# SonyCSLParis/vqcpc-bach

Measured on AMD Instinct MI355X. Metric: encoder-train windows/sec (Bach 4-voice, seq=256), higher is better.
Workload: dtype f32

## Files before the change

### vqcpc_bach_amd/csrc/embed_ln.hip

```cpp
#include <stdlib.h>

#include "common.h"
#include "gemm_common.h"

namespace vq {

__global__ __launch_bounds__(256) void embed_pos_fwd_kernel(const int64_t* __restrict__ tokens, int64_t n_rows, int tpb,
                                                            int nv, const float* __restrict__ table, int vmax, int dlin,
                                                            const float* __restrict__ chan, const float* __restrict__ ev,
                                                            int pos, float* __restrict__ out) {
    const int d = dlin + (ev ? 2 : 1) * pos;
    const int d4 = d >> 2;
    const int64_t total = n_rows * d4;
    int64_t e = (int64_t)blockIdx.x * blockDim.x + threadIdx.x;
    const int64_t step = (int64_t)gridDim.x * blockDim.x;
    for (; e < total; e += step) {
        const int64_t row = e / d4;
        const int col = (int)(e - row * d4) << 2;
        const int p = (int)(row % tpb);
        const int v = p % nv, evt = p / nv;
        float4 val;
        if (col < dlin) {
            const int64_t tok = tokens[row];
            val = *reinterpret_cast<const float4*>(table + ((int64_t)v * vmax + tok) * dlin + col);
// ... 206 lines not shown
                    const float4 rv = nt_load4(r + row * d + col);
                    xv.x += rv.x * msk[it].x;
                    xv.y += rv.y * msk[it].y;
                    xv.z += rv.z * msk[it].z;
                    xv.w += rv.w * msk[it].w;
                }
                const float4 dv = DYB16 ? nt_load4_bf16(reinterpret_cast<const unsigned short*>(dy) + row * d + col)
                                        : nt_load4(dy + row * d + col);
                xh[it] = make_float4((xv.x - mu) * rs, (xv.y - mu) * rs, (xv.z - mu) * rs, (xv.w - mu) * rs);
                gy[it] = make_float4(dv.x * gm[it].x, dv.y * gm[it].y, dv.z * gm[it].z, dv.w * gm[it].w);
                s1 += (gy[it].x + gy[it].y) + (gy[it].z + gy[it].w);
                s2 += (gy[it].x * xh[it].x + gy[it].y * xh[it].y) + (gy[it].z * xh[it].z + gy[it].w * xh[it].w);
                dg[it].x += dv.x * xh[it].x;
                dg[it].y += dv.y * xh[it].y;
                dg[it].z += dv.z * xh[it].z;
                dg[it].w += dv.w * xh[it].w;
                db[it].x += dv.x;
                db[it].y += dv.y;
                db[it].z += dv.z;
                db[it].w += dv.w;
            }
        }
        const float m1 = wave_sum(s1) * inv_d, m2 = wave_sum(s2) * inv_d;
#pragma unroll
        for (int it = 0; it < NIT; ++it) {
            const int col = lane * 4 + it * 256;
            if (it < nit && col < d) {
                float4 o;
                o.x = rs * (gy[it].x - m1 - xh[it].x * m2);
                o.y = rs * (gy[it].y - m1 - xh[it].y * m2);
                o.z = rs * (gy[it].z - m1 - xh[it].z * m2);
                o.w = rs * (gy[it].w - m1 - xh[it].w * m2);
                if (d_s) nt_store4(d_s + row * d + col, o);
                if (ds_b16) *reinterpret_cast<uint2*>(ds_b16 + row * d + col) = round4_bf16(o);
                if (MASKED && (d_r != nullptr || dr_b16 != nullptr)) {
                    o.x *= msk[it].x;
                    o.y *= msk[it].y;
                    o.z *= msk[it].z;
                    o.w *= msk[it].w;
                    if (d_r != nullptr) nt_store4(d_r + row * d + col, o);
                }
                if (dr_b16) *reinterpret_cast<uint2*>(dr_b16 + row * d + col) = round4_bf16(o);
            }
        }
    }
#pragma unroll
    for (int it = 0; it < NIT; ++it) {
        const int col = lane * 4 + it * 256;
        if (it < nit && col < d) {
            *reinterpret_cast<float4*>(&red[(wave * 2 + 0) * kRedW + col]) = dg[it];
            *reinterpret_cast<float4*>(&red[(wave * 2 + 1) * kRedW + col]) = db[it];
        }
    }
    __syncthreads();
    for (int i = threadIdx.x; i < 2 * d; i += 256) {
        const int which = i / d, col = i % d;
        float acc = 0.0f;
#pragma unroll
        for (int w = 0; w < 4; ++w) acc += red[(w * 2 + which) * kRedW + col];
        ws[(int64_t)blockIdx.x * 2 * d + i] = acc;
    }
}

__global__ __launch_bounds__(256) void embed_pos_scatter_kernel(const float* __restrict__ tmp, int nv, int64_t tab, int pos,
                                                                int nev, float* __restrict__ d_table,
                                                                float* __restrict__ d_chan, float* __restrict__ d_event) {
    const int64_t per = tab + pos + (int64_t)nev * pos;
    const int64_t i = (int64_t)blockIdx.x * 256 + threadIdx.x;
    const int64_t n1 = (int64_t)nv * (tab + pos);
    if (i < n1) {
        const int v = (int)(i / (tab + pos));
        const int64_t j = i - (int64_t)v * (tab + pos);
        const float x = tmp[(int64_t)v * per + j];
        if (j < tab) d_table[(int64_t)v * tab + j] = x;
        else d_chan[(int64_t)v * pos + (j - tab)] = x;
    } else if (i < n1 + (int64_t)nev * pos) {
        const int64_t e = i - n1;
        float acc = 0.0f;
        for (int v = 0; v < nv; ++v) acc += tmp[(int64_t)v * per + tab + pos + e];
        d_event[e] = acc;
    }
}

static int ln_blocks(int64_t M) { return (int)std::min<int64_t>(ceil_div(M, 4), 2048); }
static int ln_bwd_blocks(int64_t M, bool has_r, int d) {
    static const int cap_env = lab_env_int("VQCPC_LN_BWD_BLOCKS", 0);
    const int cap = cap_env > 0 ? cap_env : ((has_r || d > 512) ? 512 : 1024);
    return (int)std::min<int64_t>(ceil_div(M, 4), cap);
}
static int ln_bwd_blocks_max(int64_t M, int d) { return std::max(ln_bwd_blocks(M, true, d), ln_bwd_blocks(M, false, d)); }

__global__ __launch_bounds__(256) void block_table_gather_kernel(const float* __restrict__ table,
                                                                 const int64_t* __restrict__ tokens,
                                                                 float* __restrict__ out, int64_t M, int L, int C4) {
    const int64_t total = M * C4;
    for (int64_t e = (int64_t)blockIdx.x * blockDim.x + threadIdx.x; e < total; e += (int64_t)gridDim.x * blockDim.x) {
        const int64_t r = e / C4;
        const int c = (int)(e - r * C4);
        const int64_t id = tokens[r] * L + (r % L);
        reinterpret_cast<float4*>(out)[e] = reinterpret_cast<const float4*>(table)[id * C4 + c];
    }
}

constexpr int kSegU = 32;

template <bool G16>
__global__ __launch_bounds__(256) void block_table_segsum_kernel(const float* __restrict__ g,
                                                                 const int64_t* __restrict__ tokens,
                                                                 float* __restrict__ ws, int64_t n_blocks,
                                                                 int blocks_per_chunk, int L, int vmax, int C) {
    constexpr int W = G16 ? 2 : 1;
    extern __shared__ __attribute__((aligned(16))) float acc[];
    for (int i = threadIdx.x; i < vmax * 256 * W; i += 256) acc[i] = 0.0f;
    __syncthreads();
    const int ctiles = (C + 256 * W - 1) / (256 * W);
    const int ct = blockIdx.x % ctiles, p = (blockIdx.x / ctiles) % L, chunk = blockIdx.x / (ctiles * L);
    const int col = (ct * 256 + threadIdx.x) * W;
    const bool cok = col < C;
    const int64_t b0 = (int64_t)chunk * blocks_per_chunk;
    const int64_t b1 = min(b0 + blocks_per_chunk, n_blocks);
    const float* gp = g + (cok ? col : 0);
    const unsigned short* gp16 = reinterpret_cast<const unsigned short*>(g) + (cok ? col : 0);
    float* mine = acc + threadIdx.x * W;
    static_assert(kSegU <= 64, "one lane per row of a batch holds its token");
    for (int64_t b = b0; b < b1; b += kSegU) {
        float v[kSegU][W];
        const int tokv = (int)tokens[min(b + (int)(threadIdx.x & 63) % kSegU, b1 - 1) * L + p];
#pragma unroll
        for (int u = 0; u < kSegU; ++u) {
            const int64_t row = min(b + u, b1 - 1) * L + p;
            if constexpr (G16) {
                const uint32_t t = *reinterpret_cast<const uint32_t*>(gp16 + row * C);
                v[u][0] = b + u < b1 ? __uint_as_float(t << 16) : 0.0f;
                v[u][W - 1] = b + u < b1 ? __uint_as_float(t & 0xFFFF0000u) : 0.0f;
            } else {
                v[u][0] = b + u < b1 ? gp[row * C] : 0.0f;
            }
        }
#pragma unroll
        for (int u = 0; u < kSegU; ++u) {
            float* cell = mine + __builtin_amdgcn_readlane(tokv, u) * (256 * W);
#pragma unroll
            for (int w = 0; w < W; ++w) cell[w] += v[u][w];
        }
    }
    __syncthreads();
    if (cok) {
        float* dst = ws + (int64_t)chunk * vmax * L * C;
        for (int t = 0; t < vmax; ++t)
#pragma unroll
            for (int w = 0; w < W; ++w) dst[((int64_t)t * L + p) * C + col + w] = acc[(t * 256 + threadIdx.x) * W + w];
    }
}

__global__ __launch_bounds__(256) void embedding_bwd_kernel(const float* __restrict__ g, int64_t ldg,
                                                            const int64_t* __restrict__ sorted_idx,
                                                            const int64_t* __restrict__ perm, float* __restrict__ d_table,
                                                            int64_t M, int C) {
    constexpr int U = 8;
    const int64_t m = blockIdx.x;
    const int64_t v = sorted_idx[m];
    if (m > 0 && sorted_idx[m - 1] == v) return;
    int64_t lo = m, hi = M;
    while (lo + 1 < hi) {
        const int64_t mid = (lo + hi) >> 1;
        if (sorted_idx[mid] == v) lo = mid; else hi = mid;
    }
// ... 290 lines not shown
```

### vqcpc_bach_amd/csrc/relattn16.hip

```cpp
#include "gemm_common.h"

namespace vq {

typedef float floatx4 __attribute__((ext_vector_type(4)));

constexpr int kA16Waves = 4;
constexpr int kA16RS = 33;

__device__ __forceinline__ const float* erel16(const float* __restrict__ e1, const float* __restrict__ e2, int h, int HD,
                                               int x) {
    x = min(x, 30);
    return x < 16 ? e1 + ((int64_t)h * 16 + x) * HD : e2 + ((int64_t)h * 16 + (x - 15)) * HD;
}

__device__ __forceinline__ void wave_lds_fence() {
    __builtin_amdgcn_fence(__ATOMIC_RELEASE, "wavefront");
    __builtin_amdgcn_wave_barrier();
    __builtin_amdgcn_fence(__ATOMIC_ACQUIRE, "wavefront");
}

template <int N>
__device__ __forceinline__ void load_f4(float (&dst)[N], const float* __restrict__ p, float mul) {
#pragma unroll
    for (int v = 0; v < N / 4; ++v) {
// ... 37 lines not shown
    else store_ct<CT>(base + off, v);
}


__device__ __forceinline__ float bf16_lo(uint32_t w) { return __uint_as_float(w << 16); }
__device__ __forceinline__ float bf16_hi(uint32_t w) { return __uint_as_float(w & 0xFFFF0000u); }
template <int N, bool IN16>
__device__ __forceinline__ void load_vec(float (&dst)[N], const float* __restrict__ base, int64_t off, float mul) {
    if constexpr (!IN16) {
        load_f4<N>(dst, base + off, mul);
    } else {
        const unsigned short* p = reinterpret_cast<const unsigned short*>(base) + off;
        if constexpr (N == 4) {
            const uint2 t = *reinterpret_cast<const uint2*>(p);
            dst[0] = bf16_lo(t.x) * mul; dst[1] = bf16_hi(t.x) * mul; dst[2] = bf16_lo(t.y) * mul; dst[3] = bf16_hi(t.y) * mul;
        } else {
#pragma unroll
            for (int v = 0; v < N / 8; ++v) {
                const uint4 t = *reinterpret_cast<const uint4*>(p + 8 * v);
                dst[8 * v] = bf16_lo(t.x) * mul; dst[8 * v + 1] = bf16_hi(t.x) * mul;
                dst[8 * v + 2] = bf16_lo(t.y) * mul; dst[8 * v + 3] = bf16_hi(t.y) * mul;
                dst[8 * v + 4] = bf16_lo(t.z) * mul; dst[8 * v + 5] = bf16_hi(t.z) * mul;
                dst[8 * v + 6] = bf16_lo(t.w) * mul; dst[8 * v + 7] = bf16_hi(t.w) * mul;
            }
        }
    }
}
template <int CT, bool IN16>
__device__ __forceinline__ void load_cols(float (&dst)[CT], const float* __restrict__ base, int64_t off, float mul) {
    if constexpr (!IN16) {
        load_ct<CT>(dst, base + off, mul);
    } else {
        const unsigned short* p = reinterpret_cast<const unsigned short*>(base) + off;
        if constexpr (CT == 4) {
            const uint2 t = *reinterpret_cast<const uint2*>(p);
            dst[0] = bf16_lo(t.x) * mul; dst[1] = bf16_hi(t.x) * mul; dst[2 % CT] = bf16_lo(t.y) * mul; dst[3 % CT] = bf16_hi(t.y) * mul;
        } else if constexpr (CT == 2) {
            const uint32_t t = *reinterpret_cast<const uint32_t*>(p);
            dst[0] = bf16_lo(t) * mul; dst[1 % CT] = bf16_hi(t) * mul;
        } else {
            dst[0] = __uint_as_float((uint32_t)p[0] << 16) * mul;
        }
    }
}

__device__ __forceinline__ void split8x3(const float (&x)[8], bf16x8& h, bf16x8& m, bf16x8& l) {
    uint2 h0, m0, l0, h1, m1, l1;
    split3x4(make_float4(x[0], x[1], x[2], x[3]), h0, m0, l0);
    split3x4(make_float4(x[4], x[5], x[6], x[7]), h1, m1, l1);
    h = __builtin_bit_cast(bf16x8, make_uint4(h0.x, h0.y, h1.x, h1.y));
    m = __builtin_bit_cast(bf16x8, make_uint4(m0.x, m0.y, m1.x, m1.y));
    l = __builtin_bit_cast(bf16x8, make_uint4(l0.x, l0.y, l1.x, l1.y));
}
__device__ __forceinline__ floatx4 dot32_x6(const bf16x8& ah, const bf16x8& am, const bf16x8& al, const bf16x8& bh,
                                            const bf16x8& bm, const bf16x8& bl, floatx4 acc) {
    acc = __builtin_amdgcn_mfma_f32_16x16x32_bf16(al, bh, acc, 0, 0, 0);
    acc = __builtin_amdgcn_mfma_f32_16x16x32_bf16(ah, bl, acc, 0, 0, 0);
    acc = __builtin_amdgcn_mfma_f32_16x16x32_bf16(am, bm, acc, 0, 0, 0);
    acc = __builtin_amdgcn_mfma_f32_16x16x32_bf16(am, bh, acc, 0, 0, 0);
    acc = __builtin_amdgcn_mfma_f32_16x16x32_bf16(ah, bm, acc, 0, 0, 0);
    acc = __builtin_amdgcn_mfma_f32_16x16x32_bf16(ah, bh, acc, 0, 0, 0);
    return acc;
}

__device__ __forceinline__ float grp16_sum(float v) {
    v += __shfl_xor(v, 1, 16); v += __shfl_xor(v, 2, 16); v += __shfl_xor(v, 4, 16); v += __shfl_xor(v, 8, 16);
    return v;
}
__device__ __forceinline__ float grp16_max(float v) {
    v = fmaxf(v, __shfl_xor(v, 1, 16)); v = fmaxf(v, __shfl_xor(v, 2, 16));
    v = fmaxf(v, __shfl_xor(v, 4, 16)); v = fmaxf(v, __shfl_xor(v, 8, 16));
    return v;
}

template <int HD, bool B16 = false, bool IN16 = false, bool X6 = false>
__global__ __launch_bounds__(kA16Waves * 64) void relattn16_fwd_kernel(const float* __restrict__ qkv, int64_t ldq,
                                                                       const int64_t* __restrict__ tokens,
                                                                       const float* __restrict__ e1,
                                                                       const float* __restrict__ e2, float* __restrict__ ctx,
                                                                       int64_t ldo, float* __restrict__ probs,
                                                                       int64_t total, int H, float scale, uint32_t thr,
                                                                       float inv_keep, uint64_t seed) {
    constexpr int KH = HD / 4, CT = HD / 16;
    __shared__ float lds[kA16Waves][16 * kA16RS];
    const int lane = threadIdx.x & 63, wave = threadIdx.x >> 6, g = lane >> 4, c = lane & 15;
    float* buf = lds[wave];
    const int64_t prob = min((int64_t)blockIdx.x * kA16Waves + wave, total - 1);
    const bool live = (int64_t)blockIdx.x * kA16Waves + wave < total;
    const int64_t n = prob / H;
    const int h = (int)(prob % H);
    const int d = H * HD;
    const int64_t tokv = tokens ? tokens[n * 16 + c] : 0;
    const int64_t row_c = tokens ? tokv * 16 + c : n * 16 + c;
    const int64_t ro = row_c * ldq + h * HD + g * KH;

    float qa[KH], kb[KH];
    load_vec<KH, IN16>(qa, qkv, ro, scale);
    load_vec<KH, IN16>(kb, qkv, ro + d, 1.0f);
    floatx4 s = {0.f, 0.f, 0.f, 0.f};
    if constexpr (X6 && (HD == 32 || HD == 64)) {
        constexpr int NCH = KH / 8;
        constexpr bool Q1 = IN16 && HD == 64, K1 = IN16;
        bf16x8 qh[NCH], qm[NCH], ql[NCH];
#pragma unroll
        for (int ch = 0; ch < NCH; ++ch) {
            float q8[8], k8[8];
#pragma unroll
            for (int k = 0; k < 8; ++k) { q8[k] = qa[8 * ch + k]; k8[k] = kb[8 * ch + k]; }
            bf16x8 kh_, km, kl;
            split8x3(q8, qh[ch], qm[ch], ql[ch]);
            split8x3(k8, kh_, km, kl);
            if constexpr (Q1 && K1) {
                s = __builtin_amdgcn_mfma_f32_16x16x32_bf16(qh[ch], kh_, s, 0, 0, 0);
            } else if constexpr (K1) {
                s = __builtin_amdgcn_mfma_f32_16x16x32_bf16(ql[ch], kh_, s, 0, 0, 0);
                s = __builtin_amdgcn_mfma_f32_16x16x32_bf16(qm[ch], kh_, s, 0, 0, 0);
                s = __builtin_amdgcn_mfma_f32_16x16x32_bf16(qh[ch], kh_, s, 0, 0, 0);
            } else {
                s = dot32_x6(qh[ch], qm[ch], ql[ch], kh_, km, kl, s);
            }
        }
#pragma unroll
        for (int t = 0; t < 2; ++t) {
            float eb[KH];
            load_f4<KH>(eb, erel16(e1, e2, h, HD, 16 * t + c) + g * KH, 1.0f);
            floatx4 qe = {0.f, 0.f, 0.f, 0.f};
#pragma unroll
            for (int ch = 0; ch < NCH; ++ch) {
                float e8[8];
#pragma unroll
                for (int k = 0; k < 8; ++k) e8[k] = eb[8 * ch + k];
                bf16x8 eh, em, el;
                split8x3(e8, eh, em, el);
                if constexpr (Q1) {
                    qe = __builtin_amdgcn_mfma_f32_16x16x32_bf16(qh[ch], el, qe, 0, 0, 0);
                    qe = __builtin_amdgcn_mfma_f32_16x16x32_bf16(qh[ch], em, qe, 0, 0, 0);
                    qe = __builtin_amdgcn_mfma_f32_16x16x32_bf16(qh[ch], eh, qe, 0, 0, 0);
                } else {
                    qe = dot32_x6(qh[ch], qm[ch], ql[ch], eh, em, el, qe);
                }
            }
#pragma unroll
            for (int r = 0; r < 4; ++r) buf[(4 * g + r) * kA16RS + 16 * t + c] = qe[r];
        }
    } else {
#pragma unroll
    for (int k = 0; k < KH; ++k) s = __builtin_amdgcn_mfma_f32_16x16x4f32(qa[k], kb[k], s, 0, 0, 0);
#pragma unroll
    for (int t = 0; t < 2; ++t) {
        float eb[KH];
        load_f4<KH>(eb, erel16(e1, e2, h, HD, 16 * t + c) + g * KH, 1.0f);
        floatx4 qe = {0.f, 0.f, 0.f, 0.f};
#pragma unroll
        for (int k = 0; k < KH; ++k) qe = __builtin_amdgcn_mfma_f32_16x16x4f32(qa[k], eb[k], qe, 0, 0, 0);
#pragma unroll
        for (int r = 0; r < 4; ++r) buf[(4 * g + r) * kA16RS + 16 * t + c] = qe[r];
    }
    }
    wave_lds_fence();
    float p[4], pd[4];
#pragma unroll
    for (int r = 0; r < 4; ++r) {
        const int i = 4 * g + r;
        const float v = s[r] + buf[i * kA16RS + c - i + 15];
        const float m = grp16_max(v);
        const float e = __expf(v - m);
        p[r] = e / grp16_sum(e);
        const int64_t idx = (prob * 16 + i) * 16 + c;
        if (live) probs[idx] = p[r];
        pd[r] = p[r] * drop_scale(seed, (uint64_t)idx, thr, inv_keep);
    }
    wave_lds_fence();
#pragma unroll
    for (int r = 0; r < 4; ++r) buf[(4 * g + r) * kA16RS + c] = pd[r];
    wave_lds_fence();
    floatx4 o[CT];
#pragma unroll
    for (int ct = 0; ct < CT; ++ct) o[ct] = floatx4{0.f, 0.f, 0.f, 0.f};
#pragma unroll
    for (int sidx = 0; sidx < 4; ++sidx) {
        const int j = 4 * g + sidx;
        const float pa = buf[c * kA16RS + j];
        const int64_t tj = __shfl(tokv, j, 16);
        const int64_t row_j = tokens ? tj * 16 + j : n * 16 + j;
        float vb[CT];
        load_cols<CT, IN16>(vb, qkv, row_j * ldq + 2 * d + h * HD + CT * c, 1.0f);
#pragma unroll
        for (int ct = 0; ct < CT; ++ct) o[ct] = __builtin_amdgcn_mfma_f32_16x16x4f32(pa, vb[ct], o[ct], 0, 0, 0);
    }
    if (live) {
#pragma unroll
        for (int r = 0; r < 4; ++r) {
            float v[CT];
#pragma unroll
            for (int ct = 0; ct < CT; ++ct) v[ct] = o[ct][r];
            store_out<CT, B16>(ctx, (n * 16 + 4 * g + r) * ldo + h * HD + CT * c, v);
        }
    }
}

template <int HD, bool B16 = false, bool IN16 = false>
__global__ __launch_bounds__(kA16Waves * 64) void relattn16_bwd_kernel(
    const float* __restrict__ d_ctx, int64_t ldo, const float* __restrict__ qkv, int64_t ldq,
    const int64_t* __restrict__ tokens, const float* __restrict__ probs, const float* __restrict__ e1,
    const float* __restrict__ e2, float* __restrict__ d_qkv, int64_t ldg, float* __restrict__ ws, int64_t n_blocks, int H,
    int blocks_per_chunk, float scale, uint32_t thr, float inv_keep, uint64_t seed) {
    constexpr int KH = HD / 4, CT = HD / 16;
    __shared__ float lds[kA16Waves][16 * kA16RS];
    const int lane = threadIdx.x & 63, wave = threadIdx.x >> 6, g = lane >> 4, c = lane & 15;
    float* buf = lds[wave];
    const int h = blockIdx.y;
    const int d = H * HD;
    floatx4 de[2][CT];
#pragma unroll
    for (int t = 0; t < 2; ++t)
#pragma unroll
        for (int ct = 0; ct < CT; ++ct) de[t][ct] = floatx4{0.f, 0.f, 0.f, 0.f};
    const int64_t b0 = (int64_t)blockIdx.x * blocks_per_chunk;
    const int64_t b1 = min(b0 + blocks_per_chunk, n_blocks);
    const int iters = (int)((b1 - b0 + kA16Waves - 1) / kA16Waves);
    constexpr bool kPipe = HD <= 32;
    struct Blk {
        float doa[KH], vb[KH], p[4], dob[4][CT], qb[4][CT], kb[4][CT];
    };
    auto block_of = [&](int it) { return min(b0 + (int64_t)it * kA16Waves + wave, b1 - 1); };
    auto load_tok = [&](int64_t n) -> int64_t { return tokens ? tokens[n * 16 + c] : 0; };
    auto load_blk = [&](Blk& B, int64_t n, int64_t tokv) {
        const int64_t prob = n * H + h;
        const int64_t row_c = tokens ? tokv * 16 + c : n * 16 + c;
        load_vec<KH, IN16>(B.doa, d_ctx, (n * 16 + c) * ldo + h * HD + g * KH, 1.0f);
        load_vec<KH, IN16>(B.vb, qkv, row_c * ldq + h * HD + 2 * d + g * KH, 1.0f);
#pragma unroll
        for (int r = 0; r < 4; ++r) B.p[r] = probs[(prob * 16 + 4 * g + r) * 16 + c];
#pragma unroll
        for (int sidx = 0; sidx < 4; ++sidx) {
            const int j = 4 * g + sidx;
            const int64_t tj = __shfl(tokv, j, 16);
            const int64_t row = tokens ? tj * 16 + j : n * 16 + j;
            load_cols<CT, IN16>(B.dob[sidx], d_ctx, (n * 16 + j) * ldo + h * HD + CT * c, 1.0f);
            load_cols<CT, IN16>(B.qb[sidx], qkv, row * ldq + h * HD + CT * c, scale);
            load_cols<CT, IN16>(B.kb[sidx], qkv, row * ldq + d + h * HD + CT * c, 1.0f);
        }
    };
    Blk cur;
    int64_t tok_n1 = 0;
    if (kPipe) {
        load_blk(cur, block_of(0), load_tok(block_of(0)));
        tok_n1 = load_tok(block_of(1));
    }
    for (int it = 0; it < iters; ++it) {
        const int64_t want = b0 + (int64_t)it * kA16Waves + wave;
        const bool live = want < b1;
        const int64_t n = live ? want : b1 - 1;
        const int64_t prob = n * H + h;
        Blk nxt;
        if (kPipe) {
            load_blk(nxt, block_of(it + 1), tok_n1);
            tok_n1 = load_tok(block_of(it + 2));
        } else {
            load_blk(cur, n, load_tok(n));
        }
        floatx4 dp = {0.f, 0.f, 0.f, 0.f};
#pragma unroll
        for (int k = 0; k < KH; ++k) dp = __builtin_amdgcn_mfma_f32_16x16x4f32(cur.doa[k], cur.vb[k], dp, 0, 0, 0);
        float pd[4], ds[4];
#pragma unroll
        for (int r = 0; r < 4; ++r) {
            const int64_t idx = (prob * 16 + 4 * g + r) * 16 + c;
            const float p = cur.p[r];
            const float mk = drop_scale(seed, (uint64_t)idx, thr, inv_keep);
            const float dpm = dp[r] * mk;
            pd[r] = p * mk;
            ds[r] = p * (dpm - grp16_sum(dpm * p));
        }
        floatx4 dv[CT], dk[CT], dq[CT];
#pragma unroll
        for (int ct = 0; ct < CT; ++ct) dv[ct] = dk[ct] = dq[ct] = floatx4{0.f, 0.f, 0.f, 0.f};
#pragma unroll
        for (int sidx = 0; sidx < 4; ++sidx) {
#pragma unroll
            for (int ct = 0; ct < CT; ++ct) {
                dv[ct] = __builtin_amdgcn_mfma_f32_16x16x4f32(pd[sidx], cur.dob[sidx][ct], dv[ct], 0, 0, 0);
                dk[ct] = __builtin_amdgcn_mfma_f32_16x16x4f32(ds[sidx], cur.qb[sidx][ct], dk[ct], 0, 0, 0);
            }
        }
        wave_lds_fence();
#pragma unroll
        for (int r = 0; r < 4; ++r) buf[(4 * g + r) * kA16RS + c] = ds[r];
        wave_lds_fence();
#pragma unroll
        for (int sidx = 0; sidx < 4; ++sidx) {
            const float a = buf[c * kA16RS + 4 * g + sidx];
#pragma unroll
            for (int ct = 0; ct < CT; ++ct)
                dq[ct] = __builtin_amdgcn_mfma_f32_16x16x4f32(a, cur.kb[sidx][ct], dq[ct], 0, 0, 0);
        }
#pragma unroll
        for (int xt = 0; xt < 2; ++xt)
#pragma unroll
            for (int sidx = 0; sidx < 4; ++sidx) {
                const int x = 16 * xt + 4 * g + sidx;
                const int jj = x + c - 15;
                const float a = (x <= 30 && jj >= 0 && jj < 16) ? buf[c * kA16RS + jj] : 0.0f;
                float eb2[CT];
                load_ct<CT>(eb2, erel16(e1, e2, h, HD, x) + CT * c, 1.0f);
#pragma unroll
                for (int ct = 0; ct < CT; ++ct) dq[ct] = __builtin_amdgcn_mfma_f32_16x16x4f32(a, eb2[ct], dq[ct], 0, 0, 0);
            }
        if (live) {
#pragma unroll
            for (int xt = 0; xt < 2; ++xt)
#pragma unroll
                for (int sidx = 0; sidx < 4; ++sidx) {
                    const int i = 4 * g + sidx, x = 16 * xt + c;
                    const int jj = x + i - 15;
                    const float a = (x <= 30 && jj >= 0 && jj < 16) ? buf[i * kA16RS + jj] : 0.0f;
#pragma unroll
                    for (int ct = 0; ct < CT; ++ct)
                        de[xt][ct] = __builtin_amdgcn_mfma_f32_16x16x4f32(a, cur.qb[sidx][ct], de[xt][ct], 0, 0, 0);
                }
#pragma unroll
            for (int r = 0; r < 4; ++r) {
                float vq[CT], vk[CT], vv[CT];
#pragma unroll
                for (int ct = 0; ct < CT; ++ct) {
                    vq[ct] = dq[ct][r] * scale;
                    vk[ct] = dk[ct][r];
                    vv[ct] = dv[ct][r];
                }
                const int64_t go = (n * 16 + 4 * g + r) * ldg + h * HD + CT * c;
                store_out<CT, B16>(d_qkv, go, vq);
                store_out<CT, B16>(d_qkv, go + d, vk);
                store_out<CT, B16>(d_qkv, go + 2 * d, vv);
            }
        }
        if (kPipe) cur = nxt;
    }
    float* dst = ws + (((int64_t)blockIdx.x * kA16Waves + wave) * H + h) * 31 * HD;
#pragma unroll
    for (int xt = 0; xt < 2; ++xt)
#pragma unroll
        for (int ct = 0; ct < CT; ++ct)
#pragma unroll
            for (int r = 0; r < 4; ++r) {
                const int x = 16 * xt + 4 * g + r;
                if (x <= 30) dst[x * HD + CT * c + ct] = de[xt][ct][r];
            }
}

__device__ __forceinline__ uint32_t perm_lo(uint32_t hi_src, uint32_t lo_src) { return __builtin_amdgcn_perm(hi_src, lo_src, 0x05040100u); }
__device__ __forceinline__ uint32_t perm_hi(uint32_t hi_src, uint32_t lo_src) { return __builtin_amdgcn_perm(hi_src, lo_src, 0x07060302u); }
__device__ __forceinline__ void split2x4(const float (&v)[4], uint32_t& h01, uint32_t& h23, uint32_t& l01, uint32_t& l23) {
    h01 = bf16x2_rn(v[0], v[1]);
    h23 = bf16x2_rn(v[2], v[3]);
    l01 = bf16x2_rn(v[0] - bf16_lo(h01), v[1] - bf16_hi(h01));
    l23 = bf16x2_rn(v[2] - bf16_lo(h23), v[3] - bf16_hi(h23));
}
__device__ __forceinline__ bf16x8 frag8(uint32_t a, uint32_t b, uint32_t c, uint32_t d) {
    return __builtin_bit_cast(bf16x8, make_uint4(a, b, c, d));
}
__device__ __forceinline__ bf16x8 frag_from_packed(uint32_t d0, uint32_t d1, uint32_t d2, uint32_t d3) {
    return frag8(perm_hi(d1, d0), perm_hi(d3, d2), perm_lo(d1, d0), perm_lo(d3, d2));
}
template <int CT>
__device__ __forceinline__ void tr_rows4(const uint32_t (&R)[4][CT / 2], uint32_t (&T)[CT][2]) {
#pragma unroll
    for (int w = 0; w < CT / 2; ++w) {
        T[2 * w][0] = perm_lo(R[1][w], R[0][w]);
        T[2 * w][1] = perm_lo(R[3][w], R[2][w]);
        T[2 * w + 1][0] = perm_hi(R[1][w], R[0][w]);
        T[2 * w + 1][1] = perm_hi(R[3][w], R[2][w]);
    }
}
template <int CT>
__device__ __forceinline__ void load_row_b16(uint32_t (&dst)[CT / 2], const unsigned short* __restrict__ p) {
    if constexpr (CT == 4) {
        const uint2 t = *reinterpret_cast<const uint2*>(p);
        dst[0] = t.x; dst[1 % (CT / 2)] = t.y;
    } else {
        dst[0] = *reinterpret_cast<const uint32_t*>(p);
    }
}

template <int HD>
__global__ __launch_bounds__(kA16Waves * 64, 2) void relattn16_bwd_mm16_kernel(
    const unsigned short* __restrict__ d_ctx, int64_t ldo, const unsigned short* __restrict__ qkv, int64_t ldq,
    const float* __restrict__ probs, const float* __restrict__ e1, const float* __restrict__ e2,
    unsigned short* __restrict__ d_qkv, int64_t ldg, float* __restrict__ ws, int64_t n_blocks, int H, int blocks_per_chunk,
    float scale, uint32_t thr, float inv_keep, uint64_t seed) {
    static_assert(HD == 32 || HD == 64, "head_dim 32 / 64");
    constexpr int KH = HD / 4, CT = HD / 16, NCH = HD / 32;
    __shared__ uint32_t lds[kA16Waves][16 * kA16RS];
    const int lane = threadIdx.x & 63, wave = threadIdx.x >> 6, g = lane >> 4, c = lane & 15;
    uint32_t* buf = lds[wave];
    const int h = blockIdx.y;
    const int d = H * HD;
    const floatx4 zero4 = {0.f, 0.f, 0.f, 0.f};
    __shared__ uint4 erel_lds[2 * CT][64];
#pragma unroll
    for (int xt = 0; xt < 2; ++xt) {
        float ev[4][CT];
#pragma unroll
        for (int e = 0; e < 4; ++e) load_ct<CT>(ev[e], erel16(e1, e2, h, HD, 16 * xt + 4 * g + e) + CT * c, 1.0f);
#pragma unroll
        for (int ct = 0; ct < CT; ++ct) {
            const float v[4] = {ev[0][ct], ev[1][ct], ev[2][ct], ev[3][ct]};
            uint4 pk;
            split2x4(v, pk.x, pk.y, pk.z, pk.w);
            erel_lds[xt * CT + ct][lane] = pk;
        }
    }
    wave_lds_fence();
    floatx4 de[2][CT];
#pragma unroll
    for (int t = 0; t < 2; ++t)
#pragma unroll
        for (int ct = 0; ct < CT; ++ct) de[t][ct] = zero4;
    const int64_t b0 = (int64_t)blockIdx.x * blocks_per_chunk;
    const int64_t b1 = min(b0 + blocks_per_chunk, n_blocks);
// ... 65 lines not shown
        buf[(4 * g + 0) * kA16RS + c] = perm_lo(sh01, sl01);
        buf[(4 * g + 1) * kA16RS + c] = perm_hi(sh01, sl01);
        buf[(4 * g + 2) * kA16RS + c] = perm_lo(sh23, sl23);
        buf[(4 * g + 3) * kA16RS + c] = perm_hi(sh23, sl23);
        wave_lds_fence();
        {
            const uint32_t* rowp = buf + c * kA16RS + 4 * g;
            const bf16x8 a = frag_from_packed(rowp[0], rowp[1], rowp[2], rowp[3]);
#pragma unroll
            for (int ct = 0; ct < CT; ++ct)
                dq[ct] = __builtin_amdgcn_mfma_f32_16x16x32_bf16(a, frag8(tk[ct][0], tk[ct][1], tk[ct][0], tk[ct][1]), zero4, 0, 0, 0);
        }
#pragma unroll
        for (int xt = 0; xt < 2; ++xt) {
            uint32_t dd[4];
#pragma unroll
            for (int e = 0; e < 4; ++e) {
                const int x = 16 * xt + 4 * g + e;
                const int jj = x + c - 15;
                const bool ok = x <= 30 && jj >= 0 && jj < 16;
                const uint32_t t = buf[c * kA16RS + (ok ? jj : 0)];
                dd[e] = ok ? t : 0u;
            }
            const bf16x8 a = frag_from_packed(dd[0], dd[1], dd[2], dd[3]);
#pragma unroll
            for (int ct = 0; ct < CT; ++ct) {
                const uint4 ep = erel_lds[xt * CT + ct][lane];
                dq[ct] = __builtin_amdgcn_mfma_f32_16x16x32_bf16(a, frag8(ep.x, ep.y, ep.x, ep.y), dq[ct], 0, 0, 0);
                dq[ct] = __builtin_amdgcn_mfma_f32_16x16x32_bf16(a, frag8(ep.z, ep.w, 0u, 0u), dq[ct], 0, 0, 0);
            }
        }
        if (live) {
#pragma unroll
            for (int xt = 0; xt < 2; ++xt) {
                uint32_t dd[4];
#pragma unroll
                for (int e = 0; e < 4; ++e) {
                    const int i = 4 * g + e, x = 16 * xt + c;
                    const int jj = x + i - 15;
                    const bool ok = x <= 30 && jj >= 0 && jj < 16;
                    const uint32_t t = buf[i * kA16RS + (ok ? jj : 0)];
                    dd[e] = ok ? t : 0u;
                }
                const bf16x8 a = frag_from_packed(dd[0], dd[1], dd[2], dd[3]);
#pragma unroll
                for (int ct = 0; ct < CT; ++ct)
                    de[xt][ct] = __builtin_amdgcn_mfma_f32_16x16x32_bf16(a, frag8(tq[ct][0], tq[ct][1], tq[ct][0], tq[ct][1]),
                                                                        de[xt][ct], 0, 0, 0);
            }
#pragma unroll
            for (int r = 0; r < 4; ++r) {
                float vq[CT], vk[CT], vv[CT];
#pragma unroll
                for (int ct = 0; ct < CT; ++ct) {
                    vq[ct] = dq[ct][r] * scale;
                    vk[ct] = dk[ct][r] * scale;
                    vv[ct] = dv[ct][r];
                }
                const int64_t go = (n * 16 + 4 * g + r) * ldg + h * HD + CT * c;
                store_ct_b16<CT>(d_qkv + go, vq);
                store_ct_b16<CT>(d_qkv + go + d, vk);
                store_ct_b16<CT>(d_qkv + go + 2 * d, vv);
            }
        }
        cur = nxt;
    }
    float* dst = ws + (((int64_t)blockIdx.x * kA16Waves + wave) * H + h) * 31 * HD;
#pragma unroll
    for (int xt = 0; xt < 2; ++xt)
#pragma unroll
        for (int ct = 0; ct < CT; ++ct)
#pragma unroll
            for (int r = 0; r < 4; ++r) {
                const int x = 16 * xt + 4 * g + r;
                if (x <= 30) dst[x * HD + CT * c + ct] = de[xt][ct][r] * scale;
            }
}

static int a16_blocks_per_chunk(int64_t n_blocks, int H) {
    const int64_t chunks = std::max<int64_t>(1, std::min<int64_t>(ceil_div(n_blocks, kA16Waves), 2048 / std::max(H, 1)));
    return (int)ceil_div(n_blocks, chunks);
}

bool relattn16_supported(int H, int hd) { return H >= 1 && (hd == 16 || hd == 32 || hd == 64); }

int64_t relattn16_bwd_workspace(int64_t n_blocks, int H, int hd) {
    const int bpc = a16_blocks_per_chunk(n_blocks, H);
    const int64_t chunks = ceil_div(n_blocks, bpc);
    return (chunks * kA16Waves + 1) * H * 31 * hd * (int64_t)sizeof(float);
}

template <int HD, bool B16 = false, bool IN16 = false>
static int a16_fwd_t(const float* qkv, int64_t ldq, const int64_t* tokens, const float* e1, const float* e2, float* ctx,
                     int64_t ldo, float* probs, int64_t n_blocks, int H, float drop_p, uint64_t seed, hipStream_t s) {
    const int64_t total = n_blocks * H;
    static const int x6 = lab_env_int("VQCPC_RELATTN16_X6", 1);
    if ((HD == 32 || HD == 64) && x6 && vqcpc_gemm_get_mode() != 0) {
        hipLaunchKernelGGL((relattn16_fwd_kernel<HD, B16, IN16, (HD == 32 || HD == 64)>), dim3((unsigned)ceil_div(total, kA16Waves)), dim3(kA16Waves * 64),
                           0, s, qkv, ldq, tokens, e1, e2, ctx, ldo, probs, total, H, 1.0f / sqrtf((float)HD), drop_threshold(drop_p),
                           1.0f / (1.0f - drop_p), seed);
        VQ_CHECK_LAUNCH("relattn16_fwd (x6)");
        return VQCPC_OK;
    }
    hipLaunchKernelGGL((relattn16_fwd_kernel<HD, B16, IN16>), dim3((unsigned)ceil_div(total, kA16Waves)), dim3(kA16Waves * 64), 0, s, qkv,
                       ldq, tokens, e1, e2, ctx, ldo, probs, total, H, 1.0f / sqrtf((float)HD), drop_threshold(drop_p),
                       1.0f / (1.0f - drop_p), seed);
    VQ_CHECK_LAUNCH("relattn16_fwd");
    return VQCPC_OK;
}

template <int HD, bool B16 = false, bool IN16 = false>
static int a16_bwd_t(const float* d_ctx, int64_t ldo, const float* qkv, int64_t ldq, const int64_t* tokens,
                     const float* probs, const float* e1, const float* e2, float* d_qkv, int64_t ldg, float* ws,
                     int64_t n_blocks, int H, float drop_p, uint64_t seed, hipStream_t s, int* nsplit) {
    const int bpc = a16_blocks_per_chunk(n_blocks, H);
    const int chunks = (int)ceil_div(n_blocks, bpc);
    if constexpr (B16 && IN16 && (HD == 32 || HD == 64)) {
        static const int mm16 = lab_env_int("VQCPC_RELATTN16_MM16", 1);
        if (mm16 && tokens == nullptr && vqcpc_gemm_get_mode() != 0) {
            hipLaunchKernelGGL((relattn16_bwd_mm16_kernel<HD>), dim3(chunks, H), dim3(kA16Waves * 64), 0, s,
                               reinterpret_cast<const unsigned short*>(d_ctx), ldo, reinterpret_cast<const unsigned short*>(qkv), ldq,
                               probs, e1, e2, reinterpret_cast<unsigned short*>(d_qkv), ldg, ws, n_blocks, H, bpc,
                               1.0f / sqrtf((float)HD), drop_threshold(drop_p), 1.0f / (1.0f - drop_p), seed);
            VQ_CHECK_LAUNCH("relattn16_bwd (mm16)");
            *nsplit = chunks * kA16Waves;
            return VQCPC_OK;
        }
    }
    hipLaunchKernelGGL((relattn16_bwd_kernel<HD, B16, IN16>), dim3(chunks, H), dim3(kA16Waves * 64), 0, s, d_ctx, ldo, qkv, ldq, tokens,
                       probs, e1, e2, d_qkv, ldg, ws, n_blocks, H, bpc, 1.0f / sqrtf((float)HD), drop_threshold(drop_p),
                       1.0f / (1.0f - drop_p), seed);
    VQ_CHECK_LAUNCH("relattn16_bwd");
    *nsplit = chunks * kA16Waves;
    return VQCPC_OK;
}

int relattn16_fwd(const float* qkv, int64_t ldq, const int64_t* tokens, const float* e1, const float* e2, float* ctx,
                  int64_t ldo, float* probs, int64_t n_blocks, int H, int hd, float drop_p, uint64_t seed, hipStream_t s) {
    if (hd == 16) return a16_fwd_t<16>(qkv, ldq, tokens, e1, e2, ctx, ldo, probs, n_blocks, H, drop_p, seed, s);
    if (hd == 32) return a16_fwd_t<32>(qkv, ldq, tokens, e1, e2, ctx, ldo, probs, n_blocks, H, drop_p, seed, s);
    return a16_fwd_t<64>(qkv, ldq, tokens, e1, e2, ctx, ldo, probs, n_blocks, H, drop_p, seed, s);
}

int relattn16_bwd(const float* d_ctx, int64_t ldo, const float* qkv, int64_t ldq, const int64_t* tokens, const float* probs,
                  const float* e1, const float* e2, float* d_qkv, int64_t ldg, float* ws, int64_t n_blocks, int H, int hd,
                  float drop_p, uint64_t seed, hipStream_t s, int* nsplit) {
    if (hd == 16)
        return a16_bwd_t<16>(d_ctx, ldo, qkv, ldq, tokens, probs, e1, e2, d_qkv, ldg, ws, n_blocks, H, drop_p, seed, s, nsplit);
    if (hd == 32)
        return a16_bwd_t<32>(d_ctx, ldo, qkv, ldq, tokens, probs, e1, e2, d_qkv, ldg, ws, n_blocks, H, drop_p, seed, s, nsplit);
    return a16_bwd_t<64>(d_ctx, ldo, qkv, ldq, tokens, probs, e1, e2, d_qkv, ldg, ws, n_blocks, H, drop_p, seed, s, nsplit);
}

int relattn16_fwd_b16(const float* qkv, int64_t ldq, const int64_t* tokens, const float* e1, const float* e2, void* ctx_b16,
                      int64_t ldo, float* probs, int64_t n_blocks, int H, int hd, float drop_p, uint64_t seed, hipStream_t s) {
    float* c = reinterpret_cast<float*>(ctx_b16);
    if (hd == 16) return a16_fwd_t<16, true>(qkv, ldq, tokens, e1, e2, c, ldo, probs, n_blocks, H, drop_p, seed, s);
    if (hd == 32) return a16_fwd_t<32, true>(qkv, ldq, tokens, e1, e2, c, ldo, probs, n_blocks, H, drop_p, seed, s);
    return a16_fwd_t<64, true>(qkv, ldq, tokens, e1, e2, c, ldo, probs, n_blocks, H, drop_p, seed, s);
}

int relattn16_bwd_b16(const float* d_ctx, int64_t ldo, const float* qkv, int64_t ldq, const int64_t* tokens, const float* probs,
                      const float* e1, const float* e2, void* d_qkv_b16, int64_t ldg, float* ws, int64_t n_blocks, int H, int hd,
                      float drop_p, uint64_t seed, hipStream_t s, int* nsplit) {
    float* g = reinterpret_cast<float*>(d_qkv_b16);
    if (hd == 16)
        return a16_bwd_t<16, true>(d_ctx, ldo, qkv, ldq, tokens, probs, e1, e2, g, ldg, ws, n_blocks, H, drop_p, seed, s, nsplit);
    if (hd == 32)
        return a16_bwd_t<32, true>(d_ctx, ldo, qkv, ldq, tokens, probs, e1, e2, g, ldg, ws, n_blocks, H, drop_p, seed, s, nsplit);
    return a16_bwd_t<64, true>(d_ctx, ldo, qkv, ldq, tokens, probs, e1, e2, g, ldg, ws, n_blocks, H, drop_p, seed, s, nsplit);
}

int relattn16_fwd_b16io(const void* qkv_b16, int64_t ldq, const float* e1, const float* e2, void* ctx_b16, int64_t ldo,
                        float* probs, int64_t n_blocks, int H, int hd, float drop_p, uint64_t seed, hipStream_t s) {
    const float* q = reinterpret_cast<const float*>(qkv_b16);
    float* c = reinterpret_cast<float*>(ctx_b16);
    if (hd == 16) return a16_fwd_t<16, true, true>(q, ldq, nullptr, e1, e2, c, ldo, probs, n_blocks, H, drop_p, seed, s);
    if (hd == 32) return a16_fwd_t<32, true, true>(q, ldq, nullptr, e1, e2, c, ldo, probs, n_blocks, H, drop_p, seed, s);
    return a16_fwd_t<64, true, true>(q, ldq, nullptr, e1, e2, c, ldo, probs, n_blocks, H, drop_p, seed, s);
}

int relattn16_bwd_b16io(const void* d_ctx_b16, int64_t ldo, const void* qkv_b16, int64_t ldq, const float* probs,
                        const float* e1, const float* e2, void* d_qkv_b16, int64_t ldg, float* ws, int64_t n_blocks, int H,
                        int hd, float drop_p, uint64_t seed, hipStream_t s, int* nsplit) {
    const float* dc = reinterpret_cast<const float*>(d_ctx_b16);
    const float* q = reinterpret_cast<const float*>(qkv_b16);
    float* g = reinterpret_cast<float*>(d_qkv_b16);
// ... 9 lines not shown
```

Baseline: 11620.

## Hoist relative-position embeddings into registers with persistent grid-stride waves in relattn16

```diff
diff --git a/vqcpc_bach_amd/csrc/embed_ln.hip b/vqcpc_bach_amd/csrc/embed_ln.hip
--- a/vqcpc_bach_amd/csrc/embed_ln.hip
+++ b/vqcpc_bach_amd/csrc/embed_ln.hip
@@ -312,7 +312,10 @@
     }
 }
 
-static int ln_blocks(int64_t M) { return (int)std::min<int64_t>(ceil_div(M, 4), 2048); }
+static int ln_blocks(int64_t M) {
+    static const int cap_env = lab_env_int("VQCPC_LN_FWD_BLOCKS", 0);
+    return (int)std::min<int64_t>(ceil_div(M, 4), cap_env > 0 ? cap_env : 2048);
+}
 static int ln_bwd_blocks(int64_t M, bool has_r, int d) {
     static const int cap_env = lab_env_int("VQCPC_LN_BWD_BLOCKS", 0);
     const int cap = cap_env > 0 ? cap_env : ((has_r || d > 512) ? 512 : 1024);
diff --git a/vqcpc_bach_amd/csrc/relattn16.hip b/vqcpc_bach_amd/csrc/relattn16.hip
--- a/vqcpc_bach_amd/csrc/relattn16.hip
+++ b/vqcpc_bach_amd/csrc/relattn16.hip
@@ -143,14 +143,35 @@
                                                                        int64_t total, int H, float scale, uint32_t thr,
                                                                        float inv_keep, uint64_t seed) {
     constexpr int KH = HD / 4, CT = HD / 16;
+    constexpr bool kX6 = X6 && (HD == 32 || HD == 64);
+    constexpr bool kKeepE = HD <= 32;
+    constexpr int NCH = KH >= 8 ? KH / 8 : 1;
     __shared__ float lds[kA16Waves][16 * kA16RS];
     const int lane = threadIdx.x & 63, wave = threadIdx.x >> 6, g = lane >> 4, c = lane & 15;
     float* buf = lds[wave];
-    const int64_t prob = min((int64_t)blockIdx.x * kA16Waves + wave, total - 1);
-    const bool live = (int64_t)blockIdx.x * kA16Waves + wave < total;
+    const int64_t nw = (int64_t)gridDim.x * kA16Waves, w = (int64_t)blockIdx.x * kA16Waves + wave;
+    if (w >= total) return;
+    const int h = (int)(w % H);
+    const int d = H * HD;
+    float ebk[2][KH];
+    bf16x8 ehk[2][NCH], emk[2][NCH], elk[2][NCH];
+    if constexpr (kKeepE) {
+#pragma unroll
+        for (int t = 0; t < 2; ++t) {
+            load_f4<KH>(ebk[t], erel16(e1, e2, h, HD, 16 * t + c) + g * KH, 1.0f);
+            if constexpr (kX6) {
+#pragma unroll
+                for (int ch = 0; ch < NCH; ++ch) {
+                    float e8[8];
+#pragma unroll
+                    for (int k = 0; k < 8; ++k) e8[k] = ebk[t][(8 * ch + k) % KH];
+                    split8x3(e8, ehk[t][ch], emk[t][ch], elk[t][ch]);
+                }
+            }
+        }
+    }
+    auto one = [&](int64_t prob) __attribute__((always_inline)) {
     const int64_t n = prob / H;
-    const int h = (int)(prob % H);
-    const int d = H * HD;
     const int64_t tokv = tokens ? tokens[n * 16 + c] : 0;
     const int64_t row_c = tokens ? tokv * 16 + c : n * 16 + c;
     const int64_t ro = row_c * ldq + h * HD + g * KH;
@@ -159,15 +180,15 @@
     load_vec<KH, IN16>(qa, qkv, ro, scale);
     load_vec<KH, IN16>(kb, qkv, ro + d, 1.0f);
     floatx4 s = {0.f, 0.f, 0.f, 0.f};
-    if constexpr (X6 && (HD == 32 || HD == 64)) {
-        constexpr int NCH = KH / 8;
+    wave_lds_fence();
+    if constexpr (kX6) {
         constexpr bool Q1 = IN16 && HD == 64, K1 = IN16;
         bf16x8 qh[NCH], qm[NCH], ql[NCH];
 #pragma unroll
         for (int ch = 0; ch < NCH; ++ch) {
             float q8[8], k8[8];
 #pragma unroll
-            for (int k = 0; k < 8; ++k) { q8[k] = qa[8 * ch + k]; k8[k] = kb[8 * ch + k]; }
+            for (int k = 0; k < 8; ++k) { q8[k] = qa[(8 * ch + k) % KH]; k8[k] = kb[(8 * ch + k) % KH]; }
             bf16x8 kh_, km, kl;
             split8x3(q8, qh[ch], qm[ch], ql[ch]);
             split8x3(k8, kh_, km, kl);
@@ -184,15 +205,19 @@
 #pragma unroll
         for (int t = 0; t < 2; ++t) {
             float eb[KH];
-            load_f4<KH>(eb, erel16(e1, e2, h, HD, 16 * t + c) + g * KH, 1.0f);
+            if constexpr (!kKeepE) load_f4<KH>(eb, erel16(e1, e2, h, HD, 16 * t + c) + g * KH, 1.0f);
             floatx4 qe = {0.f, 0.f, 0.f, 0.f};
 #pragma unroll
             for (int ch = 0; ch < NCH; ++ch) {
-                float e8[8];
-#pragma unroll
-                for (int k = 0; k < 8; ++k) e8[k] = eb[8 * ch + k];
                 bf16x8 eh, em, el;
-                split8x3(e8, eh, em, el);
+                if constexpr (kKeepE) {
+                    eh = ehk[t][ch]; em = emk[t][ch]; el = elk[t][ch];
+                } else {
+                    float e8[8];
+#pragma unroll
+                    for (int k = 0; k < 8; ++k) e8[k] = eb[(8 * ch + k) % KH];
+                    split8x3(e8, eh, em, el);
+                }
                 if constexpr (Q1) {
                     qe = __builtin_amdgcn_mfma_f32_16x16x32_bf16(qh[ch], el, qe, 0, 0, 0);
                     qe = __builtin_amdgcn_mfma_f32_16x16x32_bf16(qh[ch], em, qe, 0, 0, 0);
@@ -210,7 +235,12 @@
 #pragma unroll
     for (int t = 0; t < 2; ++t) {
         float eb[KH];
-        load_f4<KH>(eb, erel16(e1, e2, h, HD, 16 * t + c) + g * KH, 1.0f);
+        if constexpr (kKeepE) {
+#pragma unroll
+            for (int k = 0; k < KH; ++k) eb[k] = ebk[t][k];
+        } else {
+            load_f4<KH>(eb, erel16(e1, e2, h, HD, 16 * t + c) + g * KH, 1.0f);
+        }
         floatx4 qe = {0.f, 0.f, 0.f, 0.f};
 #pragma unroll
         for (int k = 0; k < KH; ++k) qe = __builtin_amdgcn_mfma_f32_16x16x4f32(qa[k], eb[k], qe, 0, 0, 0);
@@ -228,7 +258,7 @@
         const float e = __expf(v - m);
         p[r] = e / grp16_sum(e);
         const int64_t idx = (prob * 16 + i) * 16 + c;
-        if (live) probs[idx] = p[r];
+        probs[idx] = p[r];
         pd[r] = p[r] * drop_scale(seed, (uint64_t)idx, thr, inv_keep);
     }
     wave_lds_fence();
@@ -249,19 +279,23 @@
 #pragma unroll
         for (int ct = 0; ct < CT; ++ct) o[ct] = __builtin_amdgcn_mfma_f32_16x16x4f32(pa, vb[ct], o[ct], 0, 0, 0);
     }
-    if (live) {
-#pragma unroll
-        for (int r = 0; r < 4; ++r) {
-            float v[CT];
-#pragma unroll
-            for (int ct = 0; ct < CT; ++ct) v[ct] = o[ct][r];
-            store_out<CT, B16>(ctx, (n * 16 + 4 * g + r) * ldo + h * HD + CT * c, v);
-        }
+#pragma unroll
+    for (int r = 0; r < 4; ++r) {
+        float v[CT];
+#pragma unroll
+        for (int ct = 0; ct < CT; ++ct) v[ct] = o[ct][r];
+        store_out<CT, B16>(ctx, (n * 16 + 4 * g + r) * ldo + h * HD + CT * c, v);
+    }
+    };
+    if constexpr (kKeepE) {
+        for (int64_t prob = w; prob < total; prob += nw) one(prob);
+    } else {
+        one(w);
     }
 }
 
 template <int HD, bool B16 = false, bool IN16 = false>
-__global__ __launch_bounds__(kA16Waves * 64) void relattn16_bwd_kernel(
+__global__ __launch_bounds__(kA16Waves * 64, HD <= 32 ? 2 : 1) void relattn16_bwd_kernel(
     const float* __restrict__ d_ctx, int64_t ldo, const float* __restrict__ qkv, int64_t ldq,
     const int64_t* __restrict__ tokens, const float* __restrict__ probs, const float* __restrict__ e1,
     const float* __restrict__ e2, float* __restrict__ d_qkv, int64_t ldg, float* __restrict__ ws, int64_t n_blocks, int H,
@@ -279,7 +313,7 @@
         for (int ct = 0; ct < CT; ++ct) de[t][ct] = floatx4{0.f, 0.f, 0.f, 0.f};
     const int64_t b0 = (int64_t)blockIdx.x * blocks_per_chunk;
     const int64_t b1 = min(b0 + blocks_per_chunk, n_blocks);
-    const int iters = (int)((b1 - b0 + kA16Waves - 1) / kA16Waves);
+    const int iters = b0 + wave < b1 ? (int)((b1 - b0 - wave + kA16Waves - 1) / kA16Waves) : 0;
     constexpr bool kPipe = HD <= 32;
     struct Blk {
         float doa[KH], vb[KH], p[4], dob[4][CT], qb[4][CT], kb[4][CT];
@@ -303,18 +337,17 @@
             load_cols<CT, IN16>(B.kb[sidx], qkv, row * ldq + d + h * HD + CT * c, 1.0f);
         }
     };
-    Blk cur;
+    float erel[2][4][CT];
+    if constexpr (kPipe) {
+#pragma unroll
+        for (int xt = 0; xt < 2; ++xt)
+#pragma unroll
+            for (int sidx = 0; sidx < 4; ++sidx) load_ct<CT>(erel[xt][sidx], erel16(e1, e2, h, HD, 16 * xt + 4 * g + sidx) + CT * c, 1.0f);
+    }
     int64_t tok_n1 = 0;
-    if (kPipe) {
-        load_blk(cur, block_of(0), load_tok(block_of(0)));
-        tok_n1 = load_tok(block_of(1));
-    }
-    for (int it = 0; it < iters; ++it) {
-        const int64_t want = b0 + (int64_t)it * kA16Waves + wave;
-        const bool live = want < b1;
-        const int64_t n = live ? want : b1 - 1;
+    auto step = [&](int it, Blk& cur, Blk& nxt) __attribute__((always_inline)) {
+        const int64_t n = b0 + (int64_t)it * kA16Waves + wave;
         const int64_t prob = n * H + h;
-        Blk nxt;
         if (kPipe) {
             load_blk(nxt, block_of(it + 1), tok_n1);
             tok_n1 = load_tok(block_of(it + 2));
@@ -364,11 +397,16 @@
                 const int jj = x + c - 15;
                 const float a = (x <= 30 && jj >= 0 && jj < 16) ? buf[c * kA16RS + jj] : 0.0f;
                 float eb2[CT];
-                load_ct<CT>(eb2, erel16(e1, e2, h, HD, x) + CT * c, 1.0f);
+                if constexpr (kPipe) {
+#pragma unroll
+                    for (int ct = 0; ct < CT; ++ct) eb2[ct] = erel[xt][sidx][ct];
+                } else {
+                    load_ct<CT>(eb2, erel16(e1, e2, h, HD, x) + CT * c, 1.0f);
+                }
 #pragma unroll
                 for (int ct = 0; ct < CT; ++ct) dq[ct] = __builtin_amdgcn_mfma_f32_16x16x4f32(a, eb2[ct], dq[ct], 0, 0, 0);
             }
-        if (live) {
+        {
 #pragma unroll
             for (int xt = 0; xt < 2; ++xt)
 #pragma unroll
@@ -395,7 +433,26 @@
                 store_out<CT, B16>(d_qkv, go + 2 * d, vv);
             }
         }
-        if (kPipe) cur = nxt;
+    };
+    if constexpr (kPipe) {
+        Blk opa, opb;
+        load_blk(opa, block_of(0), load_tok(block_of(0)));
+        tok_n1 = load_tok(block_of(1));
+#pragma unroll
+        for (int xt = 0; xt < 2; ++xt)
+#pragma unroll
+            for (int sidx = 0; sidx < 4; ++sidx)
+#pragma unroll
+                for (int ct = 0; ct < CT; ++ct) asm volatile("" : "+v"(erel[xt][sidx][ct]));
+        asm volatile("" : "+v"(tok_n1));
+        for (int it = 0; it < iters; it += 2) {
+            step(it, opa, opb);
+            if (it + 1 >= iters) break;
+            step(it + 1, opb, opa);
+        }
+    } else {
+        Blk cur;
+        for (int it = 0; it < iters; ++it) step(it, cur, cur);
     }
     float* dst = ws + (((int64_t)blockIdx.x * kA16Waves + wave) * H + h) * 31 * HD;
 #pragma unroll
@@ -627,6 +684,16 @@
     return (int)ceil_div(n_blocks, chunks);
 }
 
+static unsigned a16_fwd_grid(int64_t total, int H, int hd) {
+    if (hd > 32) return (unsigned)ceil_div(total, kA16Waves);
+    static const int cap = lab_env_int("VQCPC_RELATTN16_FWD_GRID", 8192);
+    int64_t grid = std::min<int64_t>(ceil_div(total, kA16Waves), cap);
+    int gcd = H, rem = kA16Waves;
+    while (rem) { const int t = gcd % rem; gcd = rem; rem = t; }
+    const int64_t unit = H / gcd;
+    return (unsigned)(ceil_div(grid, unit) * unit);
+}
+
 bool relattn16_supported(int H, int hd) { return H >= 1 && (hd == 16 || hd == 32 || hd == 64); }
 
 int64_t relattn16_bwd_workspace(int64_t n_blocks, int H, int hd) {
@@ -641,13 +708,13 @@
     const int64_t total = n_blocks * H;
     static const int x6 = lab_env_int("VQCPC_RELATTN16_X6", 1);
     if ((HD == 32 || HD == 64) && x6 && vqcpc_gemm_get_mode() != 0) {
-        hipLaunchKernelGGL((relattn16_fwd_kernel<HD, B16, IN16, (HD == 32 || HD == 64)>), dim3((unsigned)ceil_div(total, kA16Waves)), dim3(kA16Waves * 64),
+        hipLaunchKernelGGL((relattn16_fwd_kernel<HD, B16, IN16, (HD == 32 || HD == 64)>), dim3(a16_fwd_grid(total, H, HD)), dim3(kA16Waves * 64),
                            0, s, qkv, ldq, tokens, e1, e2, ctx, ldo, probs, total, H, 1.0f / sqrtf((float)HD), drop_threshold(drop_p),
                            1.0f / (1.0f - drop_p), seed);
         VQ_CHECK_LAUNCH("relattn16_fwd (x6)");
         return VQCPC_OK;
     }
-    hipLaunchKernelGGL((relattn16_fwd_kernel<HD, B16, IN16>), dim3((unsigned)ceil_div(total, kA16Waves)), dim3(kA16Waves * 64), 0, s, qkv,
+    hipLaunchKernelGGL((relattn16_fwd_kernel<HD, B16, IN16>), dim3(a16_fwd_grid(total, H, HD)), dim3(kA16Waves * 64), 0, s, qkv,
                        ldq, tokens, e1, e2, ctx, ldo, probs, total, H, 1.0f / sqrtf((float)HD), drop_threshold(drop_p),
                        1.0f / (1.0f - drop_p), seed);
     VQ_CHECK_LAUNCH("relattn16_fwd");
```

Result: no change. 11600 (-0.2%).
